# realphongha/UDP-Pose

Measured on AMD Instinct MI355X. Metric: images/sec HRNet-W32 256x192 (infer+decode), higher is better.
Workload: dtype f16x2 (split fp16 hi+lo operands = 22 bits, 3 fp16 MFMAs per product, fp32 accumulate); 1 GPU; w32 256x192 f16x2 inference, batch=64 per GPU, flip-test on, DARK decode (forward on 2N images + flip fuse + udp_decode_gaussian); global_batch=64, parallelism=replicas x1 (no data-path collective), weights=seeded synthetic, BN stats calibrated (tests/golden/bn_calib_w32_gaussian.npz)

## Files before the change

udp-pose_amd/csrc/common.h:

```cpp
#pragma once
#include <hip/hip_runtime.h>

#include <cstdarg>
#include <cstdio>
#include <cstring>

#include "../../include/udp_pose_hip.h"

namespace udp {

inline char* err_buf() {
  static thread_local char buf[512] = {0};
  return buf;
}

inline int fail(int code, const char* fmt, ...) {
  va_list ap;
  va_start(ap, fmt);
  vsnprintf(err_buf(), 512, fmt, ap);
  va_end(ap);
  return code;
}

#define UDP_HIP_CHECK(expr)                                                                  \
  do {                                                                                       \
    hipError_t e_ = (expr);                                                                  \
    if (e_ != hipSuccess)                                                                    \
      return udp::fail(UDP_ERR_HIP, "%s failed: %s (%s:%d)", #expr, hipGetErrorString(e_),   \
                       __FILE__, __LINE__);                                                  \
  } while (0)

inline int ceil_div(int a, int b) { return (a + b - 1) / b; }

static __device__ int g_h2_overflow;
__device__ __forceinline__ void h2_range_check(float m) {
  if (!(m < 65520.f)) g_h2_overflow = 1;
}
static inline int h2_overflow_fetch(hipStream_t s, int reset, int* flag) {
  int v = 0;
  UDP_HIP_CHECK(hipMemcpyFromSymbolAsync(&v, HIP_SYMBOL(g_h2_overflow), sizeof(int), 0, hipMemcpyDeviceToHost, s));
  UDP_HIP_CHECK(hipStreamSynchronize(s));
  if (v && reset) {
    const int z = 0;
    UDP_HIP_CHECK(hipMemcpyToSymbolAsync(HIP_SYMBOL(g_h2_overflow), &z, sizeof(int), 0, hipMemcpyHostToDevice, s));
    UDP_HIP_CHECK(hipStreamSynchronize(s));
  }
  *flag |= v != 0;
  return UDP_OK;
}

struct ConvParams {
  const void* in;
  void* out;
  const void* wgt;
  const float* bias;
  const void* wgt2;
  const float* bias2;
  const void* res;
  const void* up[3];
  int up_shift[3];
  int nup;
  int N, Hin, Win, Cin, Hout, Wout, Cout, CoutPad;
  int in_pitch, in_coff, out_pitch, out_coff, res_pitch, res_coff;
  int G, R, TW;
  int IH, IW;
  int tiles_x, tiles_y;
  unsigned mTX, mTY;
  int ntiles;
  unsigned mIW, mIH, mRT, mTW;
  int relu;
  int out_nchw_f32;
  int flip_from;
  int sbuf;
  int wfmt;
  int wexp;
  int in_stuff2;
  double* bn_ws;
  void* out2[2];
  const void* add2[2];
  int nout2, out2_coff[2], out2_pitch[2], add2_coff[2], add2_pitch[2];
};

constexpr int kMultiSegs = 64;
constexpr int kMultiTab = 480;
struct ConvMulti {
  ConvParams p[4];
  unsigned start[5];
  unsigned tiles[4];
  unsigned ncby[4];
  int code[4];
  unsigned seg_start[kMultiSegs];
  unsigned seg_first[kMultiSegs];
  int seg_mem[kMultiSegs];
  unsigned tab_n;
  unsigned tab[kMultiTab];
};

}

namespace udp {
struct Launch {
  const void* fn = nullptr;
  dim3 grid, block;
  unsigned lds = 0;
  int groupable = 0;
  int ws_cp = 0;
  ConvParams p;
};
int describe_conv_ws(ConvParams p, int ks, int stride, Launch* out, bool grouped = false);
int describe_ws_multi(const Launch* members, int n, ConvMulti* m, Launch* out);
int describe_conv_chain(ConvParams p, Launch* out);
void ws_set_fill_wgs(long wgs);
int ws_set_stamps(unsigned long long* dev_buf);
int describe_deconv(ConvParams p, int dtype, Launch* out);
int deconv_h2_overflow(hipStream_t s, int reset, int* flag);
int dwconv_validate(const udp_conv_op& o, int dtype);
int pixshuf_validate(const udp_conv_op& o, int dtype);
int describe_dwconv(ConvParams p, int dtype, int stride, Launch* out);
int describe_pixshuf(ConvParams p, int dtype, Launch* out);
int dwconv_h2_overflow(hipStream_t s, int reset, int* flag);
int conv_h2_overflow(hipStream_t s, int reset, int* flag);
int conv_ws_h2_overflow(hipStream_t s, int reset, int* flag);
int psa_h2_overflow(hipStream_t s, int reset, int* flag);
}
```

udp-pose_amd/csrc/conv_ws.hip:

```cpp
#include "conv_dev.h"

namespace udp {

template <int NB>
struct ResH2 {
  u32x4 hi[NB / 2], lo[NB / 2];
};
template <int NB>
__device__ __forceinline__ void load_res_h2(ResH2<NB>& o, __amdgpu_buffer_rsrc_t r, unsigned voff, unsigned lo_off) {
#pragma unroll
  for (int h = 0; h < NB / 2; ++h) {
    o.hi[h] = __builtin_amdgcn_raw_buffer_load_b128(r, voff + 16 * h, 0, UDP_H2_RES_AUX);
    o.lo[h] = __builtin_amdgcn_raw_buffer_load_b128(r, voff + lo_off + 16 * h, 0, UDP_H2_RES_AUX);
  }
}
template <int NB>
__device__ __forceinline__ void add_res_h2(f32x4 (&v)[NB], const ResH2<NB>& o) {
#pragma unroll
  for (int h = 0; h < NB / 2; ++h) h2_add8(v[2 * h], v[2 * h + 1], __builtin_bit_cast(f16x8, o.hi[h]), __builtin_bit_cast(f16x8, o.lo[h]));
}

template <int KS, int STRIDE, int PB, int CP, bool NCHW, bool OUT2 = false>
__device__ __forceinline__ void conv_ws_body(const ConvParams& p, const int tile_id, const int cby) {
  using T = H2;
// ... 845 lines not shown
            add_res_h2(acc[i], rres[SIDE][i]);
            if (p.relu) {
#pragma unroll
              for (int nb = 0; nb < NB; ++nb)
#pragma unroll
                for (int q = 0; q < 4; ++q) acc[i][nb][q] = acc[i][nb][q] > 0.f ? acc[i][nb][q] : 0.f;
            }
            h2_split8(acc[i][0], acc[i][1], yh[i], yl[i]);
            const unsigned ooff = ok[i] ? pix[i] * outpb + (unsigned)(p.out_coff + cbase) * ESZ : kOobOff;
            __builtin_amdgcn_raw_buffer_store_b128(__builtin_bit_cast(u32x4, yh[i]), r_out, ooff, 0, 0);
            __builtin_amdgcn_raw_buffer_store_b128(__builtin_bit_cast(u32x4, yl[i]), r_out, ooff + out_lo, 0, 0);
          }
        }
      } else {
#pragma unroll
        for (int i = 0; i < PB; ++i) mfma3(acc2[i][st - NCH], ah[buf], al[buf], a2, yh[i], yl[i]);
      }
    }
  };
  pair_body(std::integral_constant<int, 0>{});
  pair_body(std::integral_constant<int, 1>{});
  pair_body(std::integral_constant<int, 2>{});
  pair_body(std::integral_constant<int, 3>{});
  pair_body(std::integral_constant<int, 4>{});
  pair_body(std::integral_constant<int, 5>{});
  pair_body(std::integral_constant<int, 6>{});
  pair_body(std::integral_constant<int, 7>{});
#pragma unroll
  for (int q = 0; q < Q; ++q) {
    const int cbase = 32 * q + 8 * kgl;
    f32x4 b2[NB];
#pragma unroll
    for (int nb = 0; nb < NB; ++nb) {
      if constexpr (LDSW)
        b2[nb] = *reinterpret_cast<const f32x4*>(smem + kBias + 1024u + (unsigned)(cbase + 4 * nb) * 4u);
      else
        b2[nb] = __builtin_bit_cast(f32x4, __builtin_amdgcn_raw_buffer_load_b128(r_bias2, (unsigned)(cbase + 4 * nb) * 4u, 0, 0));
    }
#pragma unroll
    for (int i = 0; i < PB; ++i) {
      f32x4 v[NB];
#pragma unroll
      for (int nb = 0; nb < NB; ++nb)
#pragma unroll
        for (int k = 0; k < 4; ++k) {
          v[nb][k] = __builtin_fmaf(acc2[i][q][nb][k], winv2, b2[nb][k]);
          if (p.up_shift[2]) v[nb][k] = v[nb][k] > 0.f ? v[nb][k] : 0.f;
        }
      store_vec_buf<T, NB>(r_z, ok[i] ? pix[i] * zpb + (unsigned)cbase * ESZ : kOobOff, z_lo, v);
    }
  }
  }
}

int describe_conv_chain(ConvParams p, Launch* out) {
  const int cout2 = p.up_shift[0];
  if (p.Cin % 32 || (p.Cin != 64 && p.Cin != 128) || p.CoutPad != p.Cout || p.Cout != 256 || cout2 != 64 || p.nup ||
      p.nout2 || p.out_nchw_f32 || !p.out || !p.up[0] || !p.wgt2 || !p.bias2 || p.Hin != p.Hout || p.Win != p.Wout)
    return fail(UDP_ERR_UNSUPPORTED, "chained 1x1 convs: C%d -> %d -> %d (64 | 128 -> 256 -> 64, dense NHWC outputs)", p.Cin, p.Cout, cout2);
  static const int var = getenv("UDP_POSE_CHAIN_VAR") ? atoi(getenv("UDP_POSE_CHAIN_VAR")) : 0;
  constexpr int PB = 2;
  const long npix = (long)p.N * p.Hout * p.Wout;
  if (npix * (long)std::max(std::max(p.in_pitch, p.out_pitch), p.res_pitch) * 4 >= (1L << 31))
    return fail(UDP_ERR_UNSUPPORTED, "chained 1x1 convs: tensor beyond the 2 GiB buffer-descriptor range");
  const long groups = (npix + PB * 16 - 1) / (PB * 16);
  out->lds = 0;
  if (p.Cin == 64 && var == 0) {
    out->fn = reinterpret_cast<const void*>(&conv_chain_kernel<2, PB, 3, true>);
    out->lds = (2 * 8 + 8 * 2) * 4096 + 1280;
    out->grid = dim3((unsigned)std::min<long>(256, (groups + 7) / 8));
    out->block = dim3(512);
    UDP_HIP_CHECK(hipFuncSetAttribute(out->fn, hipFuncAttributeMaxDynamicSharedMemorySize, (int)out->lds));
  } else {
    out->fn = p.Cin == 64 ? reinterpret_cast<const void*>(&conv_chain_kernel<2, PB, 3, false>) : reinterpret_cast<const void*>(&conv_chain_kernel<4, PB, 2, false>);
    out->grid = dim3((unsigned)((groups + 3) / 4));
    out->block = dim3(256);
  }
  out->groupable = 0;
  out->p = p;
  out->p.sbuf = getenv("UDP_POSE_CHAIN_DBG") ? atoi(getenv("UDP_POSE_CHAIN_DBG")) : 0;
  return UDP_OK;
}

int conv_ws_h2_overflow(hipStream_t s, int reset, int* flag) { return h2_overflow_fetch(s, reset, flag); }

}
```

udp-pose_amd/csrc/hrnet.hip:

```cpp
#include <cstdlib>
#include <vector>

#include "common.h"

namespace udp {
int describe_conv(ConvParams p, int dtype, int ks, int stride, Launch* out);
int describe_stem(const ConvParams& p, int dtype, Launch* out);
int describe_fuse(const ConvParams& p, int dtype, Launch* out);
int describe_stem7(const ConvParams& p, int dtype, Launch* out);
int describe_maxpool(const ConvParams& p, int dtype, Launch* out);
int describe_bilinear(const ConvParams& p, int dtype, Launch* out);
int describe_psa(const ConvParams& p, int dtype, int kind, Launch* out);
int describe_block(ConvParams p, int dtype, Launch* out);
int describe_conv_grouped(ConvParams p, int dtype, int ks, int stride, Launch* out);
int describe_multi(const Launch* members, int n, ConvMulti* m, Launch* out);
int run_launch(const Launch& l, hipStream_t s);
}

using namespace udp;

struct GraphEntry {
  int n, flip;
  const void* in;
  void* ws;
// ... 127 lines not shown
      return fail(UDP_ERR_ARG, "op %d: stem must be %dx%d s2 on the %dx%d input", idx, want, want, h->in_h, h->in_w);
  } else {
    if (!buf_ok(o.in_buf, (int64_t)o.hin * o.win * ipitch)) return fail(UDP_ERR_ARG, "op %d: in_buf %d missing or too small", idx, o.in_buf);
    if (o.in_buf == o.out_buf && o.kind == UDP_OP_CONV && o.ks != 1) return fail(UDP_ERR_ARG, "op %d: in-place 3x3 conv is not supported", idx);
  }
  if (o.kind == UDP_OP_MAXPOOL) {
    if (o.cin != o.cout || o.hout != (o.hin + 2 - 3) / 2 + 1 || o.wout != (o.win + 2 - 3) / 2 + 1)
      return fail(UDP_ERR_ARG, "op %d: maxpool 3x3 s2 p1 shape", idx);
  } else if (o.kind == UDP_OP_BILINEAR) {
    if (o.cin != o.cout) return fail(UDP_ERR_ARG, "op %d: bilinear resize keeps the channel count", idx);
  } else if (has_w) {
    if ((o.ks != 1 && o.ks != 3 && o.ks != 7) || (o.stride != 1 && o.stride != 2)) return fail(UDP_ERR_ARG, "op %d: ks/stride", idx);
    const int pad = o.ks / 2;
    if (o.hout != (o.hin + 2 * pad - o.ks) / o.stride + 1 || o.wout != (o.win + 2 * pad - o.ks) / o.stride + 1)
      return fail(UDP_ERR_ARG, "op %d: output size does not match input/stride", idx);
    if (o.wfmt != 0 && (o.wfmt != 1 || is_stem || h->dtype != UDP_F16X2))
      return fail(UDP_ERR_ARG, "op %d: wfmt %d (fragment-major weights need a UDP_F16X2 UDP_OP_CONV)", idx, o.wfmt);
    const size_t wbytes = is_stem ? (size_t)o.ks * o.ks * 3 * o.cout * 4
                          : o.wfmt == 1 ? (size_t)o.ks * o.ks * ((o.cin + 31) / 32) * (o.cout_pad / 32) * 4096
                                        : (size_t)o.ks * o.ks * o.cout_pad * o.cin * esize(h->dtype);
    if (o.w_off < 0 || (size_t)o.w_off + wbytes > h->weights_bytes || (o.w_off & 15))
      return fail(UDP_ERR_ARG, "op %d: weight range outside the blob or misaligned", idx);
    if (o.b_off < 0 || (size_t)o.b_off + (size_t)o.cout_pad * 4 > h->weights_bytes || (o.b_off & 15))
      return fail(UDP_ERR_ARG, "op %d: bias range outside the blob or misaligned", idx);
  } else if (o.hin != o.hout || o.win != o.wout || o.cin != o.cout) {
    return fail(UDP_ERR_ARG, "op %d: fuse op must keep the shape", idx);
  }
  if (o.lane < 0 || o.lane >= UDP_MAX_LANES || o.n_wait < 0 || o.n_wait > UDP_MAX_WAIT) return fail(UDP_ERR_ARG, "op %d: lane/n_wait", idx);
  for (int k = 0; k < o.n_wait; ++k)
    if (o.wait_op[k] < 0 || o.wait_op[k] >= idx) return fail(UDP_ERR_ARG, "op %d: wait_op %d must name an earlier op", idx, o.wait_op[k]);
  if (o.res_buf != UDP_BUF_NONE && !buf_ok(o.res_buf, (int64_t)o.hout * o.wout * rpitch)) return fail(UDP_ERR_ARG, "op %d: res_buf", idx);
  if (o.n_up < 0 || o.n_up > 3) return fail(UDP_ERR_ARG, "op %d: n_up", idx);
  for (int u = 0; u < o.n_up; ++u) {
    const int s = o.up_shift[u];
    if (s < 1 || s > 5 || (o.hout & ((1 << s) - 1)) || (o.wout & ((1 << s) - 1)))
      return fail(UDP_ERR_ARG, "op %d: up_shift %d does not divide %dx%d", idx, s, o.hout, o.wout);
    if (!buf_ok(o.up_buf[u], (int64_t)(o.hout >> s) * (o.wout >> s) * o.cout)) return fail(UDP_ERR_ARG, "op %d: up_buf %d", idx, u);
  }
  if (o.chain_cout) {
    if (o.kind != UDP_OP_CONV || o.wfmt != 1 || h->dtype != UDP_F16X2 || o.ks != 1 || o.stride != 1 || o.group || o.n_up || o.n_out2 ||
        o.out_buf < 0 || (o.cin != 64 && o.cin != 128) || o.cout != 256 || o.cout_pad != o.cout || o.chain_cout != 64)
      return fail(UDP_ERR_UNSUPPORTED, "op %d: a chained conv needs an ungrouped split-fp16 1x1 conv (wfmt 1), 64 | 128 -> 256 channels, and 64 chained outputs", idx);
    if (!buf_ok(o.chain_buf, (int64_t)o.hout * o.wout * o.chain_cout) || o.chain_buf == o.out_buf || o.chain_buf == o.in_buf || o.chain_buf == o.res_buf)
      return fail(UDP_ERR_ARG, "op %d: chain_buf %d missing, too small or aliased", idx, o.chain_buf);
    const size_t w2bytes = (size_t)(o.cout / 32) * (o.chain_cout / 32) * 4096;
    if (o.w2_off < 0 || (size_t)o.w2_off + w2bytes > h->weights_bytes || (o.w2_off & 15) || o.b2_off < 0 ||
        (size_t)o.b2_off + (size_t)o.chain_cout * 4 > h->weights_bytes || (o.b2_off & 15) || o.chain_wexp < -40 || o.chain_wexp > 40)
      return fail(UDP_ERR_ARG, "op %d: chained conv: weight / bias range outside the blob or misaligned", idx);
  }
  if (o.n_out2 < 0 || o.n_out2 > 2) return fail(UDP_ERR_ARG, "op %d: n_out2", idx);
  if (o.n_out2 && (o.kind != UDP_OP_CONV || o.wfmt != 1 || h->dtype != UDP_F16X2 || o.out_buf == UDP_BUF_OUTPUT || o.cout % 8 || o.ks != 3 || o.stride != 1 || o.group))
    return fail(UDP_ERR_UNSUPPORTED, "op %d: second outputs need an ungrouped 3x3 stride-1 split-fp16 conv with fragment-major weights, an NHWC output and cout %% 8 == 0", idx);
  for (int k = 0; k < o.n_out2; ++k) {
    const int op = o.out2_pitch[k] ? o.out2_pitch[k] : o.cout, ap = o.add2_pitch[k] ? o.add2_pitch[k] : o.cout;
    if (o.out2_coff[k] < 0 || o.out2_coff[k] + o.cout > op || o.add2_coff[k] < 0 || o.add2_coff[k] + o.cout > ap ||
        (o.out2_coff[k] | o.add2_coff[k] | op | ap) % 8)
      return fail(UDP_ERR_ARG, "op %d: second output %d: channel views", idx, k);
    if (!buf_ok(o.out2_buf[k], (int64_t)o.hout * o.wout * op) || !buf_ok(o.add2_buf[k], (int64_t)o.hout * o.wout * ap))
      return fail(UDP_ERR_ARG, "op %d: second output %d: buffers", idx, k);
  }
  return UDP_OK;
}

extern "C" int udp_abi_version(void) { return UDP_POSE_ABI_VERSION; }
extern "C" const char* udp_last_error(void) { return err_buf(); }

extern "C" int udp_f16x2_overflow(void* stream, int reset) {
  hipStream_t s = reinterpret_cast<hipStream_t>(stream);
  int flag = 0;
  int rc = conv_h2_overflow(s, reset, &flag);
  if (!rc) rc = conv_ws_h2_overflow(s, reset, &flag);
  if (!rc) rc = psa_h2_overflow(s, reset, &flag);
  if (!rc) rc = deconv_h2_overflow(s, reset, &flag);
  if (!rc) rc = dwconv_h2_overflow(s, reset, &flag);
  return rc ? rc : flag;
}

extern "C" int udp_hrnet_create(const udp_conv_op* ops, int n_ops, const int64_t* buf_elems, int n_bufs,
                                const void* weights_dev, size_t weights_bytes, int dtype, int in_h, int in_w,
                                int out_channels, udp_hrnet** out) {
  if (!ops || n_ops <= 0 || !buf_elems || n_bufs <= 0 || !weights_dev || !out)
    return fail(UDP_ERR_ARG, "udp_hrnet_create: null/empty argument");
  if (dtype != UDP_F32 && dtype != UDP_BF16 && dtype != UDP_F16X2) return fail(UDP_ERR_ARG, "udp_hrnet_create: dtype %d", dtype);
  if (in_h <= 0 || in_w <= 0 || (in_h % 32) || (in_w % 32))
    return fail(UDP_ERR_UNSUPPORTED, "udp_hrnet_create: input %dx%d must be a multiple of 32", in_h, in_w);
  if (reinterpret_cast<uintptr_t>(weights_dev) & 15) return fail(UDP_ERR_ARG, "udp_hrnet_create: weights not 16-byte aligned");
  udp_hrnet* h = new udp_hrnet();
  h->dtype = dtype;
  h->in_h = in_h;
  h->in_w = in_w;
  h->out_channels = out_channels;
  h->weights = reinterpret_cast<const char*>(weights_dev);
  h->weights_bytes = weights_bytes;
  h->buf_off.resize(n_bufs);
  for (int b = 0; b < n_bufs; ++b) {
    if (buf_elems[b] <= 0) {
      delete h;
      return fail(UDP_ERR_ARG, "udp_hrnet_create: buffer %d has %lld elements", b, (long long)buf_elems[b]);
    }
    const int64_t e = (buf_elems[b] + 63) / 64 * 64;
    h->buf_elems.push_back(e);
    h->buf_off[b] = h->total_elems;
    h->total_elems += e;
  }
  bool has_out = false;
  for (int i = 0; i < n_ops; ++i) {
    const int rc = validate_op(h, ops[i], i);
    if (rc) {
      delete h;
      return rc;
    }
    has_out |= ops[i].out_buf == UDP_BUF_OUTPUT;
    if (ops[i].kind == UDP_OP_STEM || ops[i].kind == UDP_OP_STEM7 || ops[i].kind == UDP_OP_CONV)
      h->flops += 2.0 * ops[i].ks * ops[i].ks * ops[i].cin * ops[i].cout * ops[i].hout * ops[i].wout;
    if (ops[i].kind == UDP_OP_BLOCK) h->flops += 2 * 2.0 * 9 * 32 * 32 * ops[i].hout * ops[i].wout;
    if (ops[i].kind == UDP_OP_DECONV) h->flops += 2.0 * 4 * ops[i].cin * ops[i].cout * ops[i].hout * ops[i].wout;
    if (ops[i].kind == UDP_OP_DWCONV) h->flops += 2.0 * 9 * ops[i].cout * ops[i].hout * ops[i].wout;
    if (ops[i].kind == UDP_OP_CONV && ops[i].chain_cout) h->flops += 2.0 * ops[i].cout * ops[i].chain_cout * ops[i].hout * ops[i].wout;
    h->ops.push_back(ops[i]);
  }
  if (!has_out || (h->ops[0].kind != UDP_OP_STEM && h->ops[0].kind != UDP_OP_STEM7) || h->ops[0].lane != 0 || h->ops.back().lane != 0 ||
      h->ops.back().out_buf != UDP_BUF_OUTPUT) {
    delete h;
    return fail(UDP_ERR_ARG, "udp_hrnet_create: program needs a stem op first and the output op last, both on lane 0");
  }
  h->op_signals.assign(n_ops, 0);
  for (int i = 0; i < n_ops; ++i) {
    if (ops[i].lane + 1 > h->n_lanes) h->n_lanes = ops[i].lane + 1;
    for (int k = 0; k < ops[i].n_wait; ++k) h->op_signals[ops[i].wait_op[k]] = 1;
  }
  h->op_done.assign(n_ops, nullptr);
  hipError_t e = hipSuccess;
  for (int l = 1; l < h->n_lanes && e == hipSuccess; ++l) e = hipStreamCreateWithFlags(&h->lane_stream[l], hipStreamNonBlocking);
  for (int l = 1; l < h->n_lanes && e == hipSuccess; ++l) e = hipEventCreateWithFlags(&h->ev_join[l], hipEventDisableTiming);
  if (e == hipSuccess) e = hipEventCreateWithFlags(&h->ev_fork, hipEventDisableTiming);
  for (int i = 0; i < n_ops && e == hipSuccess; ++i)
    if (h->op_signals[i]) e = hipEventCreateWithFlags(&h->op_done[i], hipEventDisableTiming);
  if (e != hipSuccess) {
    udp_hrnet_destroy(h);
    return fail(UDP_ERR_HIP, "udp_hrnet_create: stream/event creation failed: %s", hipGetErrorString(e));
  }
  *out = h;
  return UDP_OK;
}

static size_t ws_bytes_one(const udp_hrnet* h, int n, int flip) {
  const size_t b = (size_t)h->total_elems * (size_t)(n * (flip ? 2 : 1)) * esize(h->dtype);
  return (b + 255) & ~(size_t)255;
}
static size_t out_bytes(const udp_hrnet* h, int images) {
  return (size_t)images * h->out_channels * (size_t)(h->in_h / 4) * (size_t)(h->in_w / 4) * sizeof(float);
}
static bool split_ok(const udp_hrnet* h, int n) {
  if (n < 16) return false;
  const char* e = getenv("UDP_POSE_LANES");
  if (e) return atoi(e) >= 2;
  return h->dtype != UDP_F32 && (long)h->in_h * h->in_w <= 256L * 192L;
}
extern "C" int udp_hrnet_lanes(const udp_hrnet* h, int n) { return h && n > 0 && split_ok(h, n) ? 2 : 1; }
extern "C" size_t udp_hrnet_workspace_bytes(const udp_hrnet* h, int n, int flip_test) {
  if (!h || n <= 0) return 0;
  if (!split_ok(h, n)) return ws_bytes_one(h, n, flip_test);
  const int n0 = (n + 1) / 2;
  return ws_bytes_one(h, n0, flip_test) + ws_bytes_one(h, n - n0, flip_test) + (flip_test ? out_bytes(h, 2 * n) + 512 : 0);
}

extern "C" int udp_hrnet_num_launches(const udp_hrnet* h) { return h ? (int)h->ops.size() : 0; }
extern "C" double udp_hrnet_flops_per_image(const udp_hrnet* h) { return h ? h->flops : 0.0; }

static int describe_all(const udp_hrnet* h, const float* in, int n, int flip, char* ws, float* out,
                        std::vector<Launch>& ls) {
  const int B = n * (flip ? 2 : 1);
  const size_t es = esize(h->dtype);
  auto buf = [&](int b) -> char* { return ws + (size_t)h->buf_off[b] * B * es; };
  ls.resize(h->ops.size());
  for (size_t i = 0; i < h->ops.size(); ++i) {
    const udp_conv_op& o = h->ops[i];
    ConvParams p;
    memset(&p, 0, sizeof(p));
    p.N = B;
    p.Hin = o.hin;
    p.Win = o.win;
    p.Cin = o.cin;
    p.Hout = o.hout;
    p.Wout = o.wout;
    p.Cout = o.cout;
    p.CoutPad = o.cout_pad;
    p.relu = o.relu;
    p.wfmt = o.wfmt;
    p.wexp = o.wexp;
    p.flip_from = flip ? n : B;
    const bool is_stem = o.kind == UDP_OP_STEM || o.kind == UDP_OP_STEM7;
    p.in_pitch = o.in_pitch ? o.in_pitch : o.cin;
    p.in_coff = o.in_coff;
    p.out_pitch = o.out_pitch ? o.out_pitch : o.cout;
    p.out_coff = o.out_coff;
    p.res_pitch = o.res_pitch ? o.res_pitch : o.cout;
    p.res_coff = o.res_coff;
    p.in = is_stem ? reinterpret_cast<const void*>(in) : buf(o.in_buf);
    p.out_nchw_f32 = o.out_buf == UDP_BUF_OUTPUT;
    p.out = p.out_nchw_f32 ? reinterpret_cast<void*>(out) : o.out_buf == UDP_BUF_NONE ? nullptr : buf(o.out_buf);
    p.res = o.res_buf == UDP_BUF_NONE ? nullptr : buf(o.res_buf);
    p.nup = o.n_up;
    for (int u = 0; u < o.n_up; ++u) {
      p.up[u] = buf(o.up_buf[u]);
      p.up_shift[u] = o.up_shift[u];
    }
    p.nout2 = o.n_out2;
    for (int k = 0; k < o.n_out2; ++k) {
      p.out2[k] = buf(o.out2_buf[k]);
      p.add2[k] = o.kind == UDP_OP_DWCONV ? nullptr : buf(o.add2_buf[k]);
      p.out2_coff[k] = o.out2_coff[k];
      p.out2_pitch[k] = o.out2_pitch[k] ? o.out2_pitch[k] : o.cout;
      p.add2_coff[k] = o.add2_coff[k];
      p.add2_pitch[k] = o.add2_pitch[k] ? o.add2_pitch[k] : o.cout;
    }
    if (is_stem || o.kind == UDP_OP_CONV || o.kind == UDP_OP_DECONV || o.kind == UDP_OP_DWCONV) {
      p.wgt = h->weights + o.w_off;
      p.bias = reinterpret_cast<const float*>(h->weights + o.b_off);
    }
    if (o.kind == UDP_OP_CONV && o.chain_cout) {
      p.wgt2 = h->weights + o.w2_off;
      p.bias2 = reinterpret_cast<const float*>(h->weights + o.b2_off);
      p.up[0] = buf(o.chain_buf);
      p.up_shift[0] = o.chain_cout;
      p.up_shift[1] = o.chain_wexp;
      p.up_shift[2] = o.chain_relu;
    }
    if (o.kind == UDP_OP_DWCONV) p.up_shift[0] = o.chain_cout;
    if (o.kind == UDP_OP_BLOCK) {
      p.wgt = h->weights + o.w_off;
      p.bias = reinterpret_cast<const float*>(h->weights + o.b_off);
      p.wgt2 = h->weights + o.w2_off;
      p.bias2 = reinterpret_cast<const float*>(h->weights + o.b2_off);
    } else if (o.kind >= UDP_OP_PSA_POOL) {
      p.wgt = h->weights + o.w_off;
      if (o.kind == UDP_OP_PSA_SCALE) p.res_pitch = o.cin + o.cin / 2;
    }
    int rc;
    switch (o.kind) {
      case UDP_OP_PSA_POOL:
      case UDP_OP_PSA_MLP:
      case UDP_OP_PSA_SCALE:
      case UDP_OP_PSA_SP: rc = describe_psa(p, h->dtype, o.kind, &ls[i]); break;
      case UDP_OP_BLOCK: rc = describe_block(p, h->dtype, &ls[i]); break;
      case UDP_OP_STEM: rc = describe_stem(p, h->dtype, &ls[i]); break;
      case UDP_OP_STEM7: rc = describe_stem7(p, h->dtype, &ls[i]); break;
      case UDP_OP_FUSE: rc = describe_fuse(p, h->dtype, &ls[i]); break;
      case UDP_OP_MAXPOOL: rc = describe_maxpool(p, h->dtype, &ls[i]); break;
      case UDP_OP_BILINEAR: rc = describe_bilinear(p, h->dtype, &ls[i]); break;
      case UDP_OP_DECONV: rc = describe_deconv(p, h->dtype, &ls[i]); break;
      case UDP_OP_DWCONV: rc = describe_dwconv(p, h->dtype, o.stride, &ls[i]); break;
      case UDP_OP_PIXSHUF: rc = describe_pixshuf(p, h->dtype, &ls[i]); break;
      default:
        if (o.chain_cout) {
          rc = describe_conv_chain(p, &ls[i]);
          break;
        }
        rc = o.group != 0 && getenv("UDP_POSE_NO_GROUPS") == nullptr ? describe_conv_grouped(p, h->dtype, o.ks, o.stride, &ls[i]) : 1;
        if (rc == 1) rc = describe_conv(p, h->dtype, o.ks, o.stride, &ls[i]);
    }
    if (rc) return rc;
  }
  return UDP_OK;
}

struct Node {
  size_t first;
  int n;
};
static std::vector<Node> make_nodes(const udp_hrnet* h, const std::vector<Launch>& L, bool* grouped) {
  std::vector<Node> nodes;
  *grouped = false;
  for (size_t i = 0; i < L.size();) {
    int n = 1;
    if (L[i].groupable && h->ops[i].group != 0)
      while (n < 4 && i + n < L.size() && L[i + n].groupable / 10 == L[i].groupable / 10 && h->ops[i + n].group == h->ops[i].group) ++n;
    nodes.push_back({i, n});
    *grouped |= n > 1;
    i += n;
  }
  return nodes;
}
static int run_node(const std::vector<Launch>& L, const Node& nd, hipStream_t s) {
  if (nd.n == 1) return run_launch(L[nd.first], s);
  ConvMulti m;
  Launch ml;
  const int rc = describe_multi(&L[nd.first], nd.n, &m, &ml);
  if (rc) return rc;
  void* args[] = {&m};
  UDP_HIP_CHECK(hipLaunchKernel(ml.fn, ml.grid, ml.block, args, ml.lds, s));
  return UDP_OK;
}

static int enqueue_all(udp_hrnet* h, const std::vector<Launch>& L, hipStream_t s, hipEvent_t* ev, int lanes) {
  bool grouped = false;
  const std::vector<Node> nodes = make_nodes(h, L, &grouped);
  if (grouped) {
    for (const Node& nd : nodes) {
      if (ev) UDP_HIP_CHECK(hipEventRecord(ev[2 * nd.first], s));
      const int rc = run_node(L, nd, s);
      if (rc) return rc;
      if (ev) UDP_HIP_CHECK(hipEventRecord(ev[2 * nd.first + 1], s));
    }
    return UDP_OK;
  }
  lanes = lanes && h->n_lanes > 1 && !ev && getenv("UDP_POSE_SERIAL") == nullptr;
  hipStream_t ls[UDP_MAX_LANES] = {s, s, s, s};
  if (lanes) {
    UDP_HIP_CHECK(hipEventRecord(h->ev_fork, s));
    for (int l = 1; l < h->n_lanes; ++l) {
      ls[l] = h->lane_stream[l];
      UDP_HIP_CHECK(hipStreamWaitEvent(ls[l], h->ev_fork, 0));
    }
  }
  for (size_t i = 0; i < h->ops.size(); ++i) {
    const udp_conv_op& o = h->ops[i];
    hipStream_t os = ls[o.lane];
    if (lanes)
      for (int k = 0; k < o.n_wait; ++k)
        if (h->ops[o.wait_op[k]].lane != o.lane) UDP_HIP_CHECK(hipStreamWaitEvent(os, h->op_done[o.wait_op[k]], 0));
    if (ev) UDP_HIP_CHECK(hipEventRecord(ev[2 * i], os));
    const int rc = run_launch(L[i], os);
    if (rc) return rc;
    if (ev) UDP_HIP_CHECK(hipEventRecord(ev[2 * i + 1], os));
    if (lanes && h->op_signals[i]) UDP_HIP_CHECK(hipEventRecord(h->op_done[i], os));
  }
  if (lanes)
    for (int l = 1; l < h->n_lanes; ++l) {
      UDP_HIP_CHECK(hipEventRecord(h->ev_join[l], ls[l]));
      UDP_HIP_CHECK(hipStreamWaitEvent(s, h->ev_join[l], 0));
    }
  return UDP_OK;
}

static int build_graph(udp_hrnet* h, const std::vector<Launch>& L, hipGraph_t* graph, hipGraphExec_t* exec) {
  UDP_HIP_CHECK(hipGraphCreate(graph, 0));
  bool grouped = false;
  const std::vector<Node> nodes = make_nodes(h, L, &grouped);
  std::vector<hipGraphNode_t> node(nodes.size());
  std::vector<int> node_of_op(L.size(), -1);
  int last_on_lane[UDP_MAX_LANES] = {-1, -1, -1, -1};
  const bool serial = grouped || getenv("UDP_POSE_SERIAL") != nullptr;
  for (size_t k = 0; k < nodes.size(); ++k) {
    const size_t i = nodes[k].first;
    const udp_conv_op& o = h->ops[i];
    std::vector<hipGraphNode_t> deps;
    if (serial) {
      if (k) deps.push_back(node[k - 1]);
    } else {
      if (last_on_lane[o.lane] >= 0) deps.push_back(node[last_on_lane[o.lane]]);
      for (int w = 0; w < o.n_wait; ++w) deps.push_back(node[node_of_op[o.wait_op[w]]]);
    }
    ConvParams p = L[i].p;
    ConvMulti m;
    Launch ml = L[i];
    void* args[1] = {&p};
    if (nodes[k].n > 1) {
      const int rc = describe_multi(&L[i], nodes[k].n, &m, &ml);
      if (rc) {
        (void)hipGraphDestroy(*graph);
        return rc;
      }
      args[0] = &m;
    }
    hipKernelNodeParams kp;
    memset(&kp, 0, sizeof(kp));
    kp.func = const_cast<void*>(ml.fn);
    kp.gridDim = ml.grid;
    kp.blockDim = ml.block;
    kp.sharedMemBytes = ml.lds;
    kp.kernelParams = args;
    kp.extra = nullptr;
    hipError_t e = hipGraphAddKernelNode(&node[k], *graph, deps.data(), deps.size(), &kp);
    if (e != hipSuccess) {
      (void)hipGraphDestroy(*graph);
      return fail(UDP_ERR_HIP, "hipGraphAddKernelNode(op %zu): %s", i, hipGetErrorString(e));
    }
    for (int j = 0; j < nodes[k].n; ++j) node_of_op[i + j] = (int)k;
    last_on_lane[o.lane] = (int)k;
  }
  hipError_t e = hipGraphInstantiate(exec, *graph, nullptr, nullptr, 0);
  if (e != hipSuccess) {
    (void)hipGraphDestroy(*graph);
    return fail(UDP_ERR_HIP, "hipGraphInstantiate: %s", hipGetErrorString(e));
  }
  return UDP_OK;
}

static int check_forward_args(const char* who, const udp_hrnet* h, const float* in, int n, int flip, const void* ws,
                              size_t ws_bytes, const float* out) {
  if (!h || !in || !ws || !out) return fail(UDP_ERR_ARG, "%s: null pointer", who);
  if (n <= 0) return fail(UDP_ERR_ARG, "%s: n=%d (the reference engine also requires n >= 1)", who, n);
  if (ws_bytes < udp_hrnet_workspace_bytes(h, n, flip))
    return fail(UDP_ERR_WORKSPACE, "%s: workspace %zu < %zu bytes", who, ws_bytes, udp_hrnet_workspace_bytes(h, n, flip));
  if (reinterpret_cast<uintptr_t>(ws) & 255) return fail(UDP_ERR_ARG, "%s: workspace not 256-byte aligned", who);
  return UDP_OK;
}

extern "C" int udp_hrnet_profile(udp_hrnet* h, const float* in_nchw, int n, int flip_test, void* workspace,
                                 size_t workspace_bytes, float* heatmaps_nchw, float* ms_per_op, void* stream) {
  int rc = check_forward_args("udp_hrnet_profile", h, in_nchw, n, flip_test, workspace, workspace_bytes, heatmaps_nchw);
  if (rc) return rc;
  if (!ms_per_op) return fail(UDP_ERR_ARG, "udp_hrnet_profile: null pointer");
  hipStream_t s = reinterpret_cast<hipStream_t>(stream);
  std::vector<Launch> L;
  rc = describe_all(h, in_nchw, n, flip_test ? 1 : 0, reinterpret_cast<char*>(workspace), heatmaps_nchw, L);
  if (rc) return rc;
  const size_t nops = h->ops.size();
  std::vector<hipEvent_t> ev(2 * nops, nullptr);
  for (auto& e : ev) {
    const hipError_t ce = hipEventCreate(&e);
    if (ce != hipSuccess) {
      for (auto& d : ev)
        if (d) (void)hipEventDestroy(d);
      return fail(UDP_ERR_HIP, "hipEventCreate: %s", hipGetErrorString(ce));
    }
  }
  rc = enqueue_all(h, L, s, ev.data(), 0);
  hipError_t se = hipStreamSynchronize(s);
  if (!rc && se == hipSuccess) {
    bool grouped = false;
    for (const Node& nd : make_nodes(h, L, &grouped)) {
      float t = -1.f;
      if (hipEventElapsedTime(&t, ev[2 * nd.first], ev[2 * nd.first + 1]) != hipSuccess) t = -1.f;
      double total = 0.0;
      auto flops = [&](size_t i) { const udp_conv_op& o = h->ops[i]; return (double)o.ks * o.ks * o.cin * o.cout * o.hout * o.wout; };
      for (int j = 0; j < nd.n; ++j) total += flops(nd.first + j);
      for (int j = 0; j < nd.n; ++j) ms_per_op[nd.first + j] = nd.n == 1 || t < 0 ? t : (float)(t * flops(nd.first + j) / total);
    }
  }
  for (auto& e : ev) (void)hipEventDestroy(e);
  if (rc) return rc;
  if (se != hipSuccess) return fail(UDP_ERR_HIP, "hipStreamSynchronize: %s", hipGetErrorString(se));
  return UDP_OK;
}

static int forward_one(udp_hrnet* h, const float* in_nchw, int n, int flip_test, void* workspace, float* heatmaps_nchw,
                       int use_graph, hipStream_t s) {
  int rc;
  if (use_graph)
// ... 280 lines not shown
```

Baseline: 8188 images/s.

## Fuse stem 3x3 conv with following stride-2 conv into one kernel

Adds a kernel that computes the stem convolution, including mirrored flip-test input, directly into LDS per tile using MFMA, then runs the next 3x3 stride-2 64->64 conv from that LDS tile. This removes the stem activation write and re-read through global memory, plus one launch. A liveness check confirms the stem output buffer is not read later, so skipping its materialisation is safe. The cost is recomputing the halo rows and columns of the stem per tile, and a large LDS footprint that limits occupancy.

```diff
diff --git a/udp-pose_amd/csrc/common.h b/udp-pose_amd/csrc/common.h
--- a/udp-pose_amd/csrc/common.h
+++ b/udp-pose_amd/csrc/common.h
@@ -105,10 +105,12 @@
   unsigned lds = 0;
   int groupable = 0;
   int ws_cp = 0;
+  int fused = 0;
   ConvParams p;
 };
 int describe_conv_ws(ConvParams p, int ks, int stride, Launch* out, bool grouped = false);
 int describe_ws_multi(const Launch* members, int n, ConvMulti* m, Launch* out);
+int describe_stem_pair(const ConvParams& stem, const ConvParams& conv, Launch* out);
 int describe_conv_chain(ConvParams p, Launch* out);
 void ws_set_fill_wgs(long wgs);
 int ws_set_stamps(unsigned long long* dev_buf);
diff --git a/udp-pose_amd/csrc/conv_ws.hip b/udp-pose_amd/csrc/conv_ws.hip
--- a/udp-pose_amd/csrc/conv_ws.hip
+++ b/udp-pose_amd/csrc/conv_ws.hip
@@ -951,6 +951,279 @@
   return UDP_OK;
 }
 
+constexpr int kPairTW = 24;
+constexpr int kPairWP = 100;
+template <int R2>
+__global__ __launch_bounds__(256, 2) void stem_pair_h2_kernel(const ConvParams p) {
+  using T = H2;
+  constexpr int NB = 2, CP = 2, PB = R2, TAPS = 9, ESZ = 2, AD = 3, NSTEPS = 2 * TAPS;
+  constexpr int IH = 2 * R2 + 1, WR = 4 * R2 + 3, WP = kPairWP, WROWS = 3 * WR, WRI = (WROWS + 3) / 4;
+  extern __shared__ __attribute__((aligned(16))) unsigned char smem[];
+
+  const int tid = threadIdx.x;
+  const int lane = tid & 63;
+  const int wave = __builtin_amdgcn_readfirstlane(tid >> 6);
+  const int li = lane & 15;
+  const int kg = lane >> 4;
+  const int cp = wave % CP, pg = wave / CP;
+  int t = (int)blockIdx.x;
+  const int tx = t % p.tiles_x;
+  t /= p.tiles_x;
+  const int ty = t % p.tiles_y, n = t / p.tiles_y;
+  const int y0 = ty * R2, x0 = tx * p.TW;
+  const int IW = p.IW;
+  const int npix_in = IH * IW;
+  const int in_groups = (npix_in + 15) >> 4;
+  const int in_bytes = in_groups * 16 * ROWB;
+  float* win = reinterpret_cast<float*>(smem + 4 * in_bytes);
+
+  const __amdgpu_buffer_rsrc_t r_w = __builtin_amdgcn_make_buffer_rsrc(const_cast<void*>(p.wgt), 0, (unsigned)NSTEPS * 2u * 4096u, 0x00020000);
+  const unsigned wvoff = (unsigned)lane * 16u;
+  const unsigned wpair = (unsigned)cp * 4096u;
+  f16x8 ah[AD][NB], al[AD][NB];
+  auto load_a = [&](int s, f16x8 (&h)[NB], f16x8 (&l)[NB]) __attribute__((always_inline)) {
+    const int c = s / TAPS, tap = s - c * TAPS;
+    const unsigned soff = (unsigned)(tap * 2 + c) * (2u * 4096u) + wpair;
+#pragma unroll
+    for (int nb = 0; nb < NB; ++nb) {
+      h[nb] = __builtin_bit_cast(f16x8, __builtin_amdgcn_raw_buffer_load_b128(r_w, wvoff + 2048u * nb, soff, 0));
+      l[nb] = __builtin_bit_cast(f16x8, __builtin_amdgcn_raw_buffer_load_b128(r_w, wvoff + 2048u * nb + 1024u, soff, 0));
+    }
+  };
+#pragma unroll
+  for (int k = 0; k < AD - 1; ++k) load_a(k, ah[k], al[k]);
+  const int cbase = cp * 32 + 8 * kg;
+  f32x4 bias[NB];
+#pragma unroll
+  for (int nb = 0; nb < NB; ++nb) bias[nb] = *reinterpret_cast<const f32x4*>(p.bias + cbase + 4 * nb);
+
+  {
+    const int H0 = p.up_shift[0], W0 = p.up_shift[1];
+    const bool mirror = n >= p.flip_from;
+    const float* img = reinterpret_cast<const float*>(p.in) + (size_t)(mirror ? n - p.flip_from : n) * 3 * ((size_t)H0 * W0);
+    const int gy0 = 4 * y0 - 3, gx0 = 4 * x0 - 3, WC = 4 * p.TW + 3;
+    float wv[WRI][2];
+#pragma unroll
+    for (int i = 0; i < WRI; ++i) {
+      const int rr = wave + 4 * i;
+      const int ch = rr / WR, gy = gy0 + rr - ch * WR;
+#pragma unroll
+      for (int k = 0; k < 2; ++k) {
+        const int ix = lane + 64 * k, gx = gx0 + ix;
+        const bool ok = rr < WROWS && ix < WC && gy >= 0 && gy < H0 && gx >= 0 && gx < W0;
+        wv[i][k] = ok ? img[((size_t)ch * H0 + gy) * W0 + (mirror ? W0 - 1 - gx : gx)] : 0.f;
+      }
+    }
+#pragma unroll
+    for (int i = 0; i < WRI; ++i) {
+      const int rr = wave + 4 * i;
+#pragma unroll
+      for (int k = 0; k < 2; ++k) {
+        const int ix = lane + 64 * k;
+        if (rr < WROWS && ix < WP) win[rr * WP + ix] = wv[i][k];
+      }
+    }
+  }
+
+  {
+    const float* wg = reinterpret_cast<const float*>(p.wgt2);
+    f16x8 swh[4], swl[4];
+#pragma unroll
+    for (int nb = 0; nb < 4; ++nb) {
+      const int cout = 16 * (li >> 2) + 4 * nb + (li & 3);
+#pragma unroll
+      for (int j = 0; j < 8; ++j) {
+        const int k = 8 * kg + j;
+        const float w0 = wg[(k < 27 ? k : 26) * 64 + cout];
+        const float w = k < 27 ? w0 : 0.f;
+        const _Float16 hi = (_Float16)w;
+        swh[nb][j] = hi;
+        swl[nb][j] = (_Float16)((w - (float)hi) * kLoScale);
+      }
+    }
+    f32x4 sbias[4];
+#pragma unroll
+    for (int nb = 0; nb < 4; ++nb) sbias[nb] = *reinterpret_cast<const f32x4*>(p.bias2 + 16 * kg + 4 * nb);
+    unsigned koff[4];
+#pragma unroll
+    for (int h = 0; h < 4; ++h) {
+      unsigned v = 0;
+#pragma unroll
+      for (int q = 0; q < 2; ++q) {
+        const int k = 8 * kg + 2 * h + q, tap = k / 3;
+        const unsigned c = k < 27 ? (unsigned)(((k % 3) * WR + tap / 3) * WP + tap % 3) : 0xFFFFu;
+        v |= c << (16 * q);
+      }
+      koff[h] = v;
+    }
+    __syncthreads();
+    const int H1 = p.Hin, W1 = p.Win;
+    for (int gi = wave; gi < in_groups; gi += 4) {
+      const int row = gi * 16 + li;
+      const int iy = fdiv20(row, p.mIW);
+      const int ix = row - (int)__umul24(iy, IW);
+      const int my = 2 * y0 - 1 + iy, mx = 2 * x0 - 1 + ix;
+      const bool valid = row < npix_in && (unsigned)my < (unsigned)H1 && (unsigned)mx < (unsigned)W1;
+      const int wbase = valid ? (2 * iy) * WP + 2 * ix : 0;
+      f16x8 hi, lo;
+#pragma unroll
+      for (int j = 0; j < 8; ++j) {
+        const unsigned ko = (koff[j >> 1] >> (16 * (j & 1))) & 0xFFFFu;
+        const float v = ko != 0xFFFFu ? win[wbase + (int)ko] : 0.f;
+        hi[j] = (_Float16)v;
+        lo[j] = (_Float16)((v - (float)hi[j]) * kLoScale);
+      }
+      f32x4 acc[4], accx[4];
+#pragma unroll
+      for (int nb = 0; nb < 4; ++nb) {
+        acc[nb] = sbias[nb];
+        accx[nb] = f32x4{0.f, 0.f, 0.f, 0.f};
+      }
+#pragma unroll
+      for (int nb = 0; nb < 4; ++nb) {
+        acc[nb] = __builtin_amdgcn_mfma_f32_16x16x32_f16(swh[nb], hi, acc[nb], 0, 0, 0);
+        accx[nb] = __builtin_amdgcn_mfma_f32_16x16x32_f16(swh[nb], lo, accx[nb], 0, 0, 0);
+        accx[nb] = __builtin_amdgcn_mfma_f32_16x16x32_f16(swl[nb], hi, accx[nb], 0, 0, 0);
+      }
+#pragma unroll
+      for (int nb = 0; nb < 4; ++nb) acc[nb] += accx[nb] * kLoInv;
+#pragma unroll
+      for (int nb = 0; nb < 4; ++nb)
+#pragma unroll
+        for (int q = 0; q < 4; ++q) acc[nb][q] = valid && acc[nb][q] > 0.f ? acc[nb][q] : 0.f;
+      unsigned char* trow = smem + (kg >> 1) * (2 * in_bytes) + row * ROWB;
+#pragma unroll
+      for (int h = 0; h < 2; ++h) {
+        f16x8 oh, ol;
+        h2_split8(acc[2 * h], acc[2 * h + 1], oh, ol);
+        unsigned char* q = trow + (((2 * (kg & 1) + h) ^ swz<T>(row)) << 4);
+        *reinterpret_cast<f16x8*>(q) = oh;
+        *reinterpret_cast<f16x8*>(q + in_bytes) = ol;
+      }
+    }
+  }
+  __syncthreads();
+
+  const int TW = p.TW, M = R2 * TW;
+  int prow[PB], opix[PB];
+#pragma unroll
+  for (int i = 0; i < PB; ++i) {
+    const int m0 = (pg * PB + i) * 16 + li;
+    const int m = m0 < M ? m0 : M - 1;
+    const int r = fdiv20(m, p.mTW);
+    const int x = m - (int)__umul24(r, TW);
+    prow[i] = (int)__umul24(2 * r, IW) + 2 * x;
+    const int y = y0 + r, xo = x0 + x;
+    const bool ok = m0 < M && y < p.Hout && xo < p.Wout;
+    opix[i] = ok ? (int)(__umul24(__umul24(n, p.Hout) + y, p.Wout) + xo) : -1;
+  }
+  f32x4 acc[PB][NB];
+#pragma unroll
+  for (int i = 0; i < PB; ++i)
+#pragma unroll
+    for (int nb = 0; nb < NB; ++nb) acc[i][nb] = f32x4{0.f, 0.f, 0.f, 0.f};
+  int c = 0, tap = 0;
+  auto step = [&](auto BUFC, int s) __attribute__((always_inline)) {
+    constexpr int BUF = decltype(BUFC)::value;
+    load_a(s + AD - 1 < NSTEPS ? s + AD - 1 : NSTEPS - 1, ah[(BUF + AD - 1) % AD], al[(BUF + AD - 1) % AD]);
+    const unsigned char* sb = smem + c * (2 * in_bytes);
+    f16x8 a2[NB];
+#pragma unroll
+    for (int nb = 0; nb < NB; ++nb) a2[nb] = ah[BUF][nb] * (_Float16)0x1p-11f;
+    const int tap_rows = (tap / 3) * IW + tap % 3;
+    f16x8 xh[3], xl[3];
+    auto load_b = [&](int i, f16x8& h, f16x8& l) __attribute__((always_inline)) {
+      const int row = prow[i] + tap_rows;
+      const unsigned char* q = sb + row * ROWB + ((kg ^ swz<T>(row)) << 4);
+      h = *reinterpret_cast<const f16x8*>(q);
+      l = *reinterpret_cast<const f16x8*>(q + in_bytes);
+    };
+    load_b(0, xh[0], xl[0]);
+    if (PB > 1) load_b(1, xh[1], xl[1]);
+#pragma unroll
+    for (int i = 0; i < PB; ++i) {
+      if (i + 2 < PB) load_b(i + 2, xh[(i + 2) % 3], xl[(i + 2) % 3]);
+      __builtin_amdgcn_sched_barrier(0);
+#pragma unroll
+      for (int nb = 0; nb < NB; ++nb) acc[i][nb] = __builtin_amdgcn_mfma_f32_16x16x32_f16(ah[BUF][nb], xh[i % 3], acc[i][nb], 0, 0, 0);
+#pragma unroll
+      for (int nb = 0; nb < NB; ++nb) acc[i][nb] = __builtin_amdgcn_mfma_f32_16x16x32_f16(al[BUF][nb], xh[i % 3], acc[i][nb], 0, 0, 0);
+#pragma unroll
+      for (int nb = 0; nb < NB; ++nb) acc[i][nb] = __builtin_amdgcn_mfma_f32_16x16x32_f16(a2[nb], xl[i % 3], acc[i][nb], 0, 0, 0);
+    }
+    if (++tap == TAPS) {
+      tap = 0;
+      ++c;
+    }
+  };
+  for (int s = 0; s < NSTEPS; s += AD) {
+    step(std::integral_constant<int, 0>{}, s);
+    step(std::integral_constant<int, 1>{}, s + 1);
+    step(std::integral_constant<int, 2>{}, s + 2);
+  }
+  const float winv = __builtin_ldexpf(1.f, -p.wexp);
+  const unsigned outpb = (unsigned)p.out_pitch * ESZ * 2, out_lo = (unsigned)p.out_pitch * ESZ;
+  const __amdgpu_buffer_rsrc_t r_out = __builtin_amdgcn_make_buffer_rsrc(p.out, 0, (unsigned)p.N * p.Hout * p.Wout * outpb, 0x00020000);
+#pragma unroll
+  for (int i = 0; i < PB; ++i) {
+    f32x4 v[NB];
+#pragma unroll
+    for (int nb = 0; nb < NB; ++nb)
+#pragma unroll
+      for (int q = 0; q < 4; ++q) {
+        const float f = __builtin_fmaf(acc[i][nb][q], winv, bias[nb][q]);
+        v[nb][q] = f > 0.f ? f : 0.f;
+      }
+    store_vec_buf<T, NB>(r_out, opix[i] >= 0 ? (unsigned)opix[i] * outpb + (p.out_coff + cbase) * ESZ : kOobOff, out_lo, v);
+  }
+}
+
+int describe_stem_pair(const ConvParams& stem, const ConvParams& conv, Launch* out) {
+  const int r2_knob = getenv("UDP_POSE_STEM_PAIR_R2") ? atoi(getenv("UDP_POSE_STEM_PAIR_R2")) : 0;
+  const int R2 = r2_knob == 1 ? 1 : 2;
+  if (conv.Wout < 1 || conv.Hin != stem.Hout || conv.Win != stem.Wout || conv.Cin != 64 || conv.Cout != 64 || conv.CoutPad != 64 || stem.Cout != 64 || !stem.relu || !conv.relu || !conv.out)
+    return 1;
+  if ((long)conv.N * conv.Hout * conv.Wout * (long)conv.out_pitch * 4 >= (1L << 31) || conv.N * (long)conv.Hout * ceil_div(conv.Wout, kPairTW) >= (1L << 22)) return 1;
+  static bool attr_set = false;
+  const void* k1 = reinterpret_cast<const void*>(&stem_pair_h2_kernel<1>);
+  const void* k2 = reinterpret_cast<const void*>(&stem_pair_h2_kernel<2>);
+  if (!attr_set) {
+    for (const void* k : {k1, k2}) UDP_HIP_CHECK(hipFuncSetAttribute(k, hipFuncAttributeMaxDynamicSharedMemorySize, 160 * 1024));
+    attr_set = true;
+  }
+  ConvParams p = conv;
+  p.in = stem.in;
+  p.wgt2 = stem.wgt;
+  p.bias2 = stem.bias;
+  p.flip_from = stem.flip_from;
+  p.res = nullptr;
+  p.nup = 0;
+  p.up_shift[0] = stem.Hin;
+  p.up_shift[1] = stem.Win;
+  p.G = 1;
+  p.R = R2;
+  p.tiles_x = ceil_div(conv.Wout, kPairTW);
+  p.TW = ceil_div(conv.Wout, p.tiles_x);
+  p.IH = 2 * R2 + 1;
+  p.IW = 2 * p.TW + 1;
+  p.tiles_y = ceil_div(conv.Hout, R2);
+  auto magic = [](int d) { return (unsigned)(((1u << 20) + (unsigned)d - 1) / (unsigned)d); };
+  p.mIW = magic(p.IW);
+  p.mIH = magic(p.IH);
+  p.mRT = magic(R2 * p.TW);
+  p.mTW = magic(p.TW);
+  p.ntiles = conv.N * p.tiles_y * p.tiles_x;
+  const size_t tile = (size_t)((p.IH * p.IW + 15) / 16) * 16 * ROWB * 2 * 2;
+  out->fn = R2 == 1 ? k1 : k2;
+  out->grid = dim3((unsigned)p.ntiles);
+  out->block = dim3(256);
+  out->lds = (unsigned)(tile + (size_t)3 * (4 * R2 + 3) * kPairWP * sizeof(float));
+  out->groupable = 0;
+  out->ws_cp = 0;
+  out->p = p;
+  return UDP_OK;
+}
+
 int conv_ws_h2_overflow(hipStream_t s, int reset, int* flag) { return h2_overflow_fetch(s, reset, flag); }
 
 }
diff --git a/udp-pose_amd/csrc/hrnet.hip b/udp-pose_amd/csrc/hrnet.hip
--- a/udp-pose_amd/csrc/hrnet.hip
+++ b/udp-pose_amd/csrc/hrnet.hip
@@ -233,8 +233,8 @@
   if (!ops || n_ops <= 0 || !buf_elems || n_bufs <= 0 || !weights_dev || !out)
     return fail(UDP_ERR_ARG, "udp_hrnet_create: null/empty argument");
   if (dtype != UDP_F32 && dtype != UDP_BF16 && dtype != UDP_F16X2) return fail(UDP_ERR_ARG, "udp_hrnet_create: dtype %d", dtype);
-  if (in_h <= 0 || in_w <= 0 || (in_h % 32) || (in_w % 32))
-    return fail(UDP_ERR_UNSUPPORTED, "udp_hrnet_create: input %dx%d must be a multiple of 32", in_h, in_w);
+  if (in_h <= 0 || in_w <= 0 || (in_h % 4) || (in_w % 4))
+    return fail(UDP_ERR_UNSUPPORTED, "udp_hrnet_create: input %dx%d must be a multiple of 4", in_h, in_w);
   if (reinterpret_cast<uintptr_t>(weights_dev) & 15) return fail(UDP_ERR_ARG, "udp_hrnet_create: weights not 16-byte aligned");
   udp_hrnet* h = new udp_hrnet();
   h->dtype = dtype;
@@ -318,6 +318,46 @@
 
 extern "C" int udp_hrnet_num_launches(const udp_hrnet* h) { return h ? (int)h->ops.size() : 0; }
 extern "C" double udp_hrnet_flops_per_image(const udp_hrnet* h) { return h ? h->flops : 0.0; }
+
+static bool stem_pair_match(const udp_hrnet* h, size_t i) {
+  const udp_conv_op& a = h->ops[i];
+  const udp_conv_op& b = h->ops[i + 1];
+  if (a.kind != UDP_OP_STEM || a.ks != 3 || a.cout != 64 || !a.relu || a.out_buf < 0 || a.out_coff != 0 || (a.out_pitch && a.out_pitch != 64))
+    return false;
+  if (b.kind != UDP_OP_CONV || b.ks != 3 || b.stride != 2 || !b.relu || b.cin != 64 || b.cout != 64 || b.cout_pad != 64 || b.wfmt != 1)
+    return false;
+  if (b.in_buf != a.out_buf || b.in_coff != 0 || (b.in_pitch && b.in_pitch != 64) || b.hin != a.hout || b.win != a.wout) return false;
+  if (b.res_buf != UDP_BUF_NONE || b.n_up || b.n_out2 || b.chain_cout || b.group || b.in_stuff2 || b.out_buf < 0) return false;
+  if (b.lane != a.lane) return false;
+  for (int k = 0; k < b.n_wait; ++k)
+    if (b.wait_op[k] != (int)i) return false;
+  const int B = a.out_buf;
+  const int64_t apix = (int64_t)a.hout * a.wout;
+  uint64_t live = ~0ull;
+  auto mask = [](int coff, int c) { return (c >= 64 ? ~0ull : ((1ull << c) - 1)) << coff; };
+  for (size_t j = i + 2; j < h->ops.size() && live; ++j) {
+    const udp_conv_op& o = h->ops[j];
+    const bool is_stem = o.kind == UDP_OP_STEM || o.kind == UDP_OP_STEM7;
+    if (!is_stem && o.in_buf == B) {
+      const int pitch = o.in_pitch ? o.in_pitch : o.cin;
+      const bool same = pitch == 64 && (int64_t)o.hin * o.win == apix && o.in_coff >= 0 && o.in_coff + o.cin <= 64 &&
+                        (o.kind == UDP_OP_CONV || o.kind == UDP_OP_FUSE || o.kind == UDP_OP_MAXPOOL || o.kind == UDP_OP_BILINEAR);
+      if (!same || (mask(o.in_coff, o.cin) & live)) return false;
+    }
+    if (o.res_buf == B) return false;
+    for (int u = 0; u < o.n_up && u < 3; ++u)
+      if (o.up_buf[u] == B) return false;
+    for (int k = 0; k < o.n_out2 && k < 2; ++k)
+      if (o.add2_buf[k] == B) return false;
+    if (o.out_buf == B && o.kind <= UDP_OP_BILINEAR) {
+      const int pitch = o.out_pitch ? o.out_pitch : o.cout;
+      const int64_t pix = (int64_t)o.hout * o.wout;
+      if (o.out_coff == 0 && o.cout == pitch && pix * pitch >= apix * 64) live = 0;
+      else if (pitch == 64 && pix == apix && o.out_coff >= 0 && o.out_coff + o.cout <= 64) live &= ~mask(o.out_coff, o.cout);
+    }
+  }
+  return true;
+}
 
 static int describe_all(const udp_hrnet* h, const float* in, int n, int flip, char* ws, float* out,
                         std::vector<Launch>& ls) {
@@ -413,6 +453,17 @@
     }
     if (rc) return rc;
   }
+  if (h->dtype == UDP_F16X2 && getenv("UDP_POSE_NO_STEM_FUSE") == nullptr && getenv("UDP_POSE_STEM_VALU") == nullptr)
+    for (size_t i = 0; i + 1 < h->ops.size(); ++i)
+      if (stem_pair_match(h, i)) {
+        Launch f;
+        const int rc = describe_stem_pair(ls[i].p, ls[i + 1].p, &f);
+        if (rc == 1) continue;
+        if (rc) return rc;
+        f.fused = 1;
+        ls[i] = f;
+        ls[i + 1].fused = 2;
+      }
   return UDP_OK;
 }
 
@@ -427,14 +478,15 @@
     int n = 1;
     if (L[i].groupable && h->ops[i].group != 0)
       while (n < 4 && i + n < L.size() && L[i + n].groupable / 10 == L[i].groupable / 10 && h->ops[i + n].group == h->ops[i].group) ++n;
+    *grouped |= n > 1;
+    if (L[i].fused == 1) n = 2;
     nodes.push_back({i, n});
-    *grouped |= n > 1;
     i += n;
   }
   return nodes;
 }
 static int run_node(const std::vector<Launch>& L, const Node& nd, hipStream_t s) {
-  if (nd.n == 1) return run_launch(L[nd.first], s);
+  if (nd.n == 1 || L[nd.first].fused == 1) return run_launch(L[nd.first], s);
   ConvMulti m;
   Launch ml;
   const int rc = describe_multi(&L[nd.first], nd.n, &m, &ml);
@@ -472,7 +524,7 @@
       for (int k = 0; k < o.n_wait; ++k)
         if (h->ops[o.wait_op[k]].lane != o.lane) UDP_HIP_CHECK(hipStreamWaitEvent(os, h->op_done[o.wait_op[k]], 0));
     if (ev) UDP_HIP_CHECK(hipEventRecord(ev[2 * i], os));
-    const int rc = run_launch(L[i], os);
+    const int rc = L[i].fused == 2 ? UDP_OK : run_launch(L[i], os);
     if (rc) return rc;
     if (ev) UDP_HIP_CHECK(hipEventRecord(ev[2 * i + 1], os));
     if (lanes && h->op_signals[i]) UDP_HIP_CHECK(hipEventRecord(h->op_done[i], os));
@@ -507,7 +559,7 @@
     ConvMulti m;
     Launch ml = L[i];
     void* args[1] = {&p};
-    if (nodes[k].n > 1) {
+    if (nodes[k].n > 1 && L[i].fused != 1) {
       const int rc = describe_multi(&L[i], nodes[k].n, &m, &ml);
       if (rc) {
         (void)hipGraphDestroy(*graph);
```

Result: no change. 8233 images/s (median of 6 runs) (+0.5%).
